# Mariachiar/Spatiotemporal-Deepfake-Detection-for-Live-Video-Calls

Measured on AMD Instinct MI355X. Metric: clips/sec (32x3x224x224), higher is better.
Workload: dtype bf16

## Files before the change

### spatiotemporal-deepfake-detection-for-live-video-calls_amd/csrc/af_conv111.hip

```cpp
#include "af_common.h"

namespace af {

struct C111Args {
    const char* in;
    const char* in2;
    const char* w;
    const char* w2;
    const float* scale;
    const float* shift;
    const char* res;
    char* out;
    int Cin, Cin2, Cout, out_ld, relu;
    int ncol;
    int T, HW, chunks;
    long long M;
    int tiles;
};

template <int NL, int NS, int D, int A = 0, int B = 0>
__device__ __forceinline__ void wait_counted(int nl, int ns) {
    if constexpr (A <= D - 1 && B <= D) {
        if (nl == A && ns == B) { wait_vmcnt<A * NL + B * NS>(); return; }
        if constexpr (B < D) wait_counted<NL, NS, D, A, B + 1>(nl, ns);
        else wait_counted<NL, NS, D, A + 1, 0>(nl, ns);
    } else {
        wait_vmcnt<0>();
    }
}

template <int DT, int KS1, int KS2, bool TPOOL, bool RES, int WC, int BM = 128, int NSLOT = 2>
__global__ __launch_bounds__(512, 1) void conv111_kernel(const C111Args a) {
    typedef Elem<DT> E;
    constexpr int EPC = E::EPC, ES = 16 / EPC;
    static_assert(EPC == 8, "16-bit storage types only");
    static_assert(WC == 64 || (WC == 32 && !TPOOL), "wave columns of 64 or 32 channels; the pooled tile order assumes 64");
    static_assert((BM == 128 || (BM == 64 && !TPOOL)) && NSLOT >= 2 && NSLOT <= 4, "tiles of 128 or 64 positions; the pooled row order assumes 128");
    constexpr int KS = KS1 + KS2, TN = WC / 16, D = NSLOT - 1;
    constexpr int NWN = 256 / WC, NWM = 8 / NWN, WPOS = BM / NWM, MT = WPOS / 16;
    constexpr int SLAB = BM * 128, STAGE = KS * SLAB;
    constexpr int PROW = WC + 4;
    constexpr int LPR = WC / 8, RPI = 64 / LPR, ITS = 16 / RPI;
    constexpr int NR = MT * ITS;
    constexpr int NPC = BM / 64;

    extern __shared__ uint4 smem[];
    const unsigned lds0 = (unsigned)(uintptr_t)(__attribute__((address_space(3))) char*)smem;
    const int tid = threadIdx.x, lane = tid & 63;
    const int wave = __builtin_amdgcn_readfirstlane(tid >> 6);
    const int frow = lane & 15, fg = lane >> 4;
    const int wn = wave % NWN, wm = wave / NWN;
    float* patch = reinterpret_cast<float*>(reinterpret_cast<char*>(smem) + NSLOT * STAGE) + wave * (16 * PROW);
    int col = blockIdx.x % a.ncol, first = blockIdx.x / a.ncol;
    const int stride = gridDim.x / a.ncol;
    if (gridDim.x % (8 * a.ncol) == 0) {
        const int xcd = blockIdx.x & 7, y = blockIdx.x >> 3;
        col = y % a.ncol;
        first = xcd + 8 * (y / a.ncol);
    }

    auto row_pixel = [&](int r) { return (r >> 6) * 32 + ((r >> 4) & 1) * 16 + (r & 15); };
    auto row_off = [&](int r) -> long long { return TPOOL ? (long long)((r >> 5) & 1) * a.HW + row_pixel(r) : r; };

    uint4 wreg[TN][2 * KS];
#pragma unroll
    for (int i = 0; i < TN; ++i) {
        const long long ch = col * 256 + wn * WC + i * 16 + frow;
#pragma unroll
        for (int k = 0; k < 2 * KS1; ++k)
            wreg[i][k] = *reinterpret_cast<const uint4*>(a.w + (ch * a.Cin + k * 32 + fg * 8) * ES);
#pragma unroll
        for (int k = 0; k < 2 * KS2; ++k)
            wreg[i][2 * KS1 + k] = *reinterpret_cast<const uint4*>(a.w2 + (ch * a.Cin2 + k * 32 + fg * 8) * ES);
    }

    constexpr bool REGEPI = WC == 32;
    const int rr = REGEPI ? frow : lane / LPR, cc = REGEPI ? (fg & 1) * 16 + (fg >> 1) * 8 : (lane % LPR) * 8;
    const int ch0 = col * 256 + wn * WC + cc;
    f32x4 sc[2], sf[2];
#pragma unroll
    for (int e = 0; e < 2; ++e) {
        const int chp = REGEPI ? col * 256 + wn * WC + e * 16 + fg * 4 : ch0 + 4 * e;
        sc[e] = *reinterpret_cast<const f32x4*>(a.scale + chp);
        sf[e] = *reinterpret_cast<const f32x4*>(a.shift + chp);
    }

    const int drow = lane >> 3, chunk = (lane & 7) ^ drow;
    const int xrow = wave * 8 + drow;
    const unsigned xoff = (unsigned)(row_off(xrow) * a.Cin * ES + chunk * 16);
    const unsigned x2off = KS2 ? (unsigned)(row_off(xrow) * a.Cin2 * ES + chunk * 16) : 0u;
    const int half_off = (int)(row_off(64) * a.Cin * ES), half2_off = (int)(row_off(64) * a.Cin2 * ES);
    auto tile_origin = [&](int tile, int& live) -> long long {
        if (TPOOL) {
            const int c = tile % a.chunks, nt = tile / a.chunks;
            live = a.HW - c * 64;
            return (long long)nt * 2 * a.HW + c * 64;
        }
        const long long o = (long long)tile * BM;
        live = (int)(a.M - o < BM ? a.M - o : BM);
        return o;
    };
    auto row_live = [&](int r, int live) { return TPOOL ? row_pixel(r) < live : r < live; };

    auto issue_tile = [&](int tile, int slot) {
        int live;
        const long long o = tile_origin(tile, live);
        const i32x4 d1 = make_desc(a.in + o * a.Cin * ES);
        const unsigned base = lds0 + slot * STAGE + wave * (8 * 128);
#pragma unroll
        for (int s = 0; s < KS1; ++s)
#pragma unroll
            for (int i = 0; i < NPC; ++i)
                blds16(row_live(xrow + 64 * i, live) ? xoff : kOutOfRange, d1, s * 128 + i * half_off, base + s * SLAB + i * (64 * 128));
        if (KS2) {
            const i32x4 d2 = make_desc(a.in2 + o * a.Cin2 * ES);
#pragma unroll
            for (int s = 0; s < KS2; ++s)
#pragma unroll
                for (int i = 0; i < NPC; ++i)
                    blds16(row_live(xrow + 64 * i, live) ? x2off : kOutOfRange, d2, s * 128 + i * half2_off, base + (KS1 + s) * SLAB + i * (64 * 128));
        }
    };
    const int row0 = wm * WPOS + rr;
    const unsigned res_lane = (unsigned)((row_off(row0) * a.Cout + ch0) * ES);
    const unsigned out_lane = (unsigned)(((long long)(TPOOL ? row_pixel(row0) : row0) * a.out_ld + ch0) * ES);
    auto k_row = [&](int k) { return (k / ITS) * 16 + (k % ITS) * RPI; };
    auto res_soff = [&](int k) { return (int)((row_off(k_row(k)) * a.Cout) * ES); };
    auto out_soff = [&](int k) { return (int)(((long long)(TPOOL ? row_pixel(k_row(k)) : k_row(k)) * a.out_ld) * ES); };
    auto load_residual = [&](int tile, u32x4 (&r)[NR]) {
        int live;
        const long long o = tile_origin(tile, live);
        const i32x4 rd = make_desc(a.res + o * a.Cout * ES);
#pragma unroll
        for (int k = 0; k < NR; ++k)
            r[k] = bload16_nt_uncounted(row_live(row0 + k_row(k), live) ? res_lane : kOutOfRange, rd, res_soff(k));
    };

    const int my_tiles = first < a.tiles ? (a.tiles - first + stride - 1) / stride : 0;
    u32x4 rs[NSLOT][NR];
#pragma unroll
    for (int u = 0; u < NSLOT; ++u)
#pragma unroll
        for (int k = 0; k < NR; ++k) rs[u][k] = u32x4{0u, 0u, 0u, 0u};
#pragma unroll
    for (int j = 0; j < D; ++j)
        if (j < my_tiles) {
            issue_tile(first + j * stride, j);
            if (RES) load_residual(first + j * stride, rs[j]);
        }
    __builtin_amdgcn_sched_barrier(0);
    constexpr int NL = KS * NPC + (RES ? NR : 0), NS = TPOOL ? NR / 2 : NR;
    static_assert((D - 1) * NL + D * NS <= 63, "vmcnt range");

    for (int q0 = 0; q0 < my_tiles; q0 += NSLOT) {
#pragma unroll
    for (int u = 0; u < NSLOT; ++u) {
        const int q = q0 + u;
        if (q >= my_tiles) break;
        const int tile = first + q * stride, slot = u;
        u32x4 (&rcur)[NR] = rs[u];
        if (D == 1) wait_vmcnt<0>();
        else {
            const int nl = my_tiles - 1 - q < D - 1 ? my_tiles - 1 - q : D - 1, ns = q < D ? q : D;
            wait_counted<NL, NS, D>(nl, ns);
        }
        __builtin_amdgcn_s_barrier();
        if (RES) {
#pragma unroll
            for (int k = 0; k < NR; ++k) asm volatile("" : "+v"(rcur[k]));
        }
        if (q + D < my_tiles) {
            issue_tile(tile + D * stride, (u + D) % NSLOT);
            if (RES) load_residual(tile + D * stride, rs[(u + D) % NSLOT]);
        }
        __builtin_amdgcn_sched_barrier(0);

        int live;
        const long long o = tile_origin(tile, live);
        const long long opos = TPOOL ? (o - o % a.HW) / 2 + o % a.HW : o;
        char* obase = a.out + opos * a.out_ld * ES;
        const uint4* xs = smem + slot * (STAGE / 16) + (wm * WPOS + frow) * 8;

#pragma unroll
        for (int h = 0; h < MT / 2; ++h) {
            f32x4 acc[TN][2];
#pragma unroll
            for (int i = 0; i < TN; ++i) { acc[i][0] = f32x4{0.f, 0.f, 0.f, 0.f}; acc[i][1] = f32x4{0.f, 0.f, 0.f, 0.f}; }
#pragma unroll
            for (int k = 0; k < 2 * KS; ++k) {
                const int c = ((k & 1) * 4 + fg) ^ (frow & 7);
                uint4 bf[2];
#pragma unroll
                for (int jl = 0; jl < 2; ++jl) bf[jl] = xs[(k >> 1) * (SLAB / 16) + (TPOOL ? h + 2 * jl : 2 * h + jl) * 16 * 8 + c];
#pragma unroll
                for (int i = 0; i < TN; ++i)
#pragma unroll
                    for (int jl = 0; jl < 2; ++jl) Mma<DT>::run(wreg[i][k], bf[jl], acc[i][jl]);
            }

            if constexpr (REGEPI) {
                const float lo = a.relu ? 0.f : -__builtin_inff();
#pragma unroll
                for (int jl = 0; jl < 2; ++jl) {
                    const int j = 2 * h + jl, row = wm * WPOS + j * 16 + rr;
                    f32x4 v0 = acc[0][jl] * sc[0] + sf[0], v1 = acc[1][jl] * sc[1] + sf[1];
                    if (RES) {
                        const u32x4 x = rcur[j];
                        const u32x2 s0 = __builtin_amdgcn_permlane16_swap(x[0], x[2], false, false);
                        const u32x2 s1 = __builtin_amdgcn_permlane16_swap(x[1], x[3], false, false);
                        const u32x2 ra = u32x2{s0[0], s1[0]}, rb = u32x2{s0[1], s1[1]};
                        v0 += Vec4<DT>::load(&ra); v1 += Vec4<DT>::load(&rb);
                    }
                    v0[0] = max_nan(v0[0], lo); v0[1] = max_nan(v0[1], lo); v0[2] = max_nan(v0[2], lo); v0[3] = max_nan(v0[3], lo);
                    v1[0] = max_nan(v1[0], lo); v1[1] = max_nan(v1[1], lo); v1[2] = max_nan(v1[2], lo); v1[3] = max_nan(v1[3], lo);
                    u32x2 p0, p1;
                    Vec4<DT>::store(&p0, v0); Vec4<DT>::store(&p1, v1);
                    const u32x4 o = swap_pair16(p0, p1);
                    if (row_live(row, live))
                        __builtin_nontemporal_store(o, reinterpret_cast<u32x4*>(obase + out_soff(j) + out_lane));
                }
                continue;
            }
            float keep[ITS][8];
#pragma unroll
            for (int jl = 0; jl < 2; ++jl) {
                const int j = TPOOL ? h + 2 * jl : 2 * h + jl;
#pragma unroll
                for (int i = 0; i < TN; ++i)
                    *reinterpret_cast<f32x4*>(patch + frow * PROW + i * 16 + fg * 4) = acc[i][jl];
                __builtin_amdgcn_wave_barrier();
#pragma unroll
                for (int it = 0; it < ITS; ++it) {
                    const int prow = it * RPI + rr, row = wm * WPOS + j * 16 + prow;
                    float v[8];
#pragma unroll
                    for (int e = 0; e < 8; e += 4) {
                        const f32x4 t = *reinterpret_cast<const f32x4*>(patch + prow * PROW + cc + e);
                        const f32x4 r = t * sc[e >> 2] + sf[e >> 2];
                        v[e] = r[0]; v[e + 1] = r[1]; v[e + 2] = r[2]; v[e + 3] = r[3];
                    }
                    if (RES) {
                        const uint4 rraw = __builtin_bit_cast(uint4, rcur[j * ITS + it]);
                        const typename E::type* re = reinterpret_cast<const typename E::type*>(&rraw);
#pragma unroll
                        for (int e = 0; e < 8; ++e) v[e] += E::to_f32(re[e]);
                    }
                    if (a.relu) {
#pragma unroll
                        for (int e = 0; e < 8; ++e) v[e] = relu_f(v[e]);
                    }
                    if (TPOOL && jl == 0) {
#pragma unroll
                        for (int e = 0; e < 8; ++e) keep[it][e] = v[e];
                        continue;
                    }
                    if (TPOOL) {
#pragma unroll
                        for (int e = 0; e < 8; ++e) v[e] = max_nan(keep[it][e], v[e]);
                    }
                    uint4 ov;
                    typename E::type* oe = reinterpret_cast<typename E::type*>(&ov);
#pragma unroll
                    for (int e = 0; e < 8; ++e) oe[e] = E::from_f32(v[e]);
                    if (row_live(row, live))
                        __builtin_nontemporal_store(__builtin_bit_cast(u32x4, ov), reinterpret_cast<u32x4*>(obase + out_soff(j * ITS + it) + out_lane));
                }
                __builtin_amdgcn_wave_barrier();
            }
        }
    }
    }
}

template <int DT, int KS1, int KS2, bool TPOOL, bool RES, int WC = 64, int BM = 128, int NSLOT = 2>
static int launch111(const C111Args& a, int blocks, hipStream_t stream) {
    const int lds = NSLOT * (KS1 + KS2) * BM * 128 + 8 * 16 * (WC + 4) * 4;
    AF_SET_MAX_LDS((&conv111_kernel<DT, KS1, KS2, TPOOL, RES, WC, BM, NSLOT>), lds, "conv111");
    hipLaunchKernelGGL((conv111_kernel<DT, KS1, KS2, TPOOL, RES, WC, BM, NSLOT>), dim3(blocks), dim3(512), lds, stream, a);
    AF_CHECK_LAUNCH("conv111_kernel");
    return AF_OK;
}

static int conv111_bm(const af_conv_desc* d) { return d->cin >= 128 ? 64 : 128; }

static long long conv111_tiles(const af_conv_desc* d, const af_conv_desc* d2, int out_ld) {
    if (d->dtype == AF_F32) return 0;
    if (d->kt != 1 || d->kh != 1 || d->kw != 1 || d->st != 1 || d->sh != 1 || d->sw != 1 || d->pt || d->ph || d->pw) return 0;
    if (d->cout % 256 != 0 || (d->tpool != 0 && d->tpool != 1)) return 0;
    if (d2) {
        if (d->cin != 64 || d2->cin != 64 || d->tpool) return 0;
        if (d2->st != 1 || d2->sh != 1 || d2->sw != 1 || d2->t != d->t || d2->h != d->h || d2->w != d->w) return 0;
    } else if (d->cin != 64 && d->cin != 128 && d->cin != 256) return 0;
    if (d->tpool && (d->cin != 64 || d->t % 2 != 0)) return 0;
    const long long hw = (long long)d->h * d->w;
    if ((hw + 128) * 128 * 2 * 2 >= (1LL << 31)) return 0;
    const int bm = conv111_bm(d);
    const long long tiles = d->tpool ? (long long)d->n * (d->t / 2) * ((hw + 63) / 64) : ((long long)d->n * d->t * hw + bm - 1) / bm;
    if (tiles >= (1LL << 30)) return 0;
    if (tiles * bm / 128 * (d->cout / 256) < 4LL * device_cus()) return 0;
    return tiles;
}

bool conv111_applies(const af_conv_desc* d, const af_conv_desc* d2, const void* residual, int out_ld) {
    if (d2 && residual) return false;
    return conv111_tiles(d, d2, out_ld) != 0;
}

int conv111_run(const af_conv_desc* d, const void* in, const void* w_packed, const af_conv_desc* d2, const void* in2,
                const void* w2_packed, const float* scale, const float* shift, const void* residual, void* out, int out_ld,
                hipStream_t stream) {
    C111Args a;
    a.in = (const char*)in; a.in2 = (const char*)in2; a.w = (const char*)w_packed; a.w2 = (const char*)w2_packed;
    a.scale = scale; a.shift = shift; a.res = (const char*)residual; a.out = (char*)out;
    a.Cin = d->cin; a.Cin2 = d2 ? d2->cin : 0; a.Cout = d->cout; a.out_ld = out_ld; a.relu = d->relu;
    a.ncol = d->cout / 256;
    a.T = d->t; a.HW = d->h * d->w; a.chunks = (a.HW + 63) / 64;
    a.M = (long long)d->n * d->t * a.HW;
    a.tiles = (int)conv111_tiles(d, d2, out_ld);
    int streams = device_cus() / a.ncol;
    if (streams > a.tiles) streams = a.tiles;
    const int blocks = streams * a.ncol;
    const bool bf = d->dtype == AF_BF16;
#define AF_C111(K1, K2, TP, RS) (bf ? launch111<AF_BF16, K1, K2, TP, RS>(a, blocks, stream) : launch111<AF_F16, K1, K2, TP, RS>(a, blocks, stream))
    if (d2) return AF_C111(1, 1, false, false);
    if (d->tpool) return residual ? AF_C111(1, 0, true, true) : AF_C111(1, 0, true, false);
    if (d->cin == 64) return residual ? AF_C111(1, 0, false, true) : AF_C111(1, 0, false, false);
    if (d->cin == 256) {
        if (env_int("AF_C111_WC64", 1) != 0)
            return residual ? (bf ? launch111<AF_BF16, 4, 0, false, true, 64, 64, 2>(a, blocks, stream) : launch111<AF_F16, 4, 0, false, true, 64, 64, 2>(a, blocks, stream))
                            : (bf ? launch111<AF_BF16, 4, 0, false, false, 64, 64, 2>(a, blocks, stream) : launch111<AF_F16, 4, 0, false, false, 64, 64, 2>(a, blocks, stream));
        return residual ? (bf ? launch111<AF_BF16, 4, 0, false, true, 32, 64, 4>(a, blocks, stream) : launch111<AF_F16, 4, 0, false, true, 32, 64, 4>(a, blocks, stream))
                        : (bf ? launch111<AF_BF16, 4, 0, false, false, 32, 64, 4>(a, blocks, stream) : launch111<AF_F16, 4, 0, false, false, 32, 64, 4>(a, blocks, stream));
    }
    return residual ? (bf ? launch111<AF_BF16, 2, 0, false, true, 64, 64, 4>(a, blocks, stream) : launch111<AF_F16, 2, 0, false, true, 64, 64, 4>(a, blocks, stream))
                    : (bf ? launch111<AF_BF16, 2, 0, false, false, 64, 64, 4>(a, blocks, stream) : launch111<AF_F16, 2, 0, false, false, 64, 64, 4>(a, blocks, stream));
#undef AF_C111
}

}
```

Measured before the change: 3499.

## Add narrow 1x1x1 conv kernel for 512-to-128 channel layers with register-resident weights

Adds a specialized persistent kernel for pointwise convolutions with 512 input and 128 output channels, a shape the existing kernel rejected because it requires cout divisible by 256. The full weight slice is held in registers per wave, activation tiles of 32 rows are streamed through a 4-slot LDS pipeline via buffer-to-LDS loads, and outputs are staged through an LDS patch for coalesced nontemporal stores. The intent is to move these layers off the slower fallback path. The cost is heavy register pressure from pinned weight fragments and a new code path to maintain.

```diff
diff --git a/spatiotemporal-deepfake-detection-for-live-video-calls_amd/csrc/af_conv111.hip b/spatiotemporal-deepfake-detection-for-live-video-calls_amd/csrc/af_conv111.hip
--- a/spatiotemporal-deepfake-detection-for-live-video-calls_amd/csrc/af_conv111.hip
+++ b/spatiotemporal-deepfake-detection-for-live-video-calls_amd/csrc/af_conv111.hip
@@ -279,6 +279,141 @@
     hipLaunchKernelGGL((conv111_kernel<DT, KS1, KS2, TPOOL, RES, WC, BM, NSLOT>), dim3(blocks), dim3(512), lds, stream, a);
     AF_CHECK_LAUNCH("conv111_kernel");
     return AF_OK;
+}
+
+template <int DT, int WC, int BM, int NSLOT>
+__global__ __launch_bounds__(512, 1) void conv111_narrow_kernel(const C111Args a) {
+    typedef Elem<DT> E;
+    static_assert(E::EPC == 8, "16-bit storage types only");
+    constexpr int K = 512, CO = 128, ROWB = K * 2, OROWB = CO * 2;
+    constexpr int TN = WC / 16, NWN = CO / WC, NWM = 8 / NWN, WPOS = BM / NWM, MT = WPOS / 16, D = NSLOT - 1;
+    static_assert((WC == 16 || WC == 32) && WPOS % 16 == 0 && MT >= 1 && BM % 8 == 0, "wave grid");
+    constexpr int STAGE = BM * ROWB, NL = BM / 8;
+    constexpr int PSTR = OROWB + 16;
+    constexpr int SB = BM * OROWB / 512, LPR = OROWB / SB, RPW = 64 / LPR;
+    static_assert((SB == 16 || SB == 8) && RPW * 8 == BM, "one store per wave and tile");
+    constexpr int NWAIT = (D - 1) * NL + D;
+    static_assert(NWAIT <= 63, "vmcnt range");
+
+    extern __shared__ uint4 smem[];
+    const unsigned lds0 = (unsigned)(uintptr_t)(__attribute__((address_space(3))) char*)smem;
+    char* const patch = reinterpret_cast<char*>(smem) + NSLOT * STAGE;
+    const int tid = threadIdx.x, lane = tid & 63;
+    const int wave = __builtin_amdgcn_readfirstlane(tid >> 6);
+    const int frow = lane & 15, fg = lane >> 4;
+    const int wn = wave % NWN, wm = wave / NWN;
+    const int first = blockIdx.x, stride = gridDim.x;
+    const int my_tiles = first < a.tiles ? (a.tiles - first + stride - 1) / stride : 0;
+
+    u32x4 wreg[TN][16];
+    f32x4 sc[TN], sf[TN];
+#pragma unroll
+    for (int i = 0; i < TN; ++i) {
+        const int ch = wn * WC + i * 16;
+#pragma unroll
+        for (int k = 0; k < 16; ++k)
+            wreg[i][k] = *reinterpret_cast<const u32x4*>(a.w + ((long long)(ch + frow) * K + k * 32 + fg * 8) * 2);
+        sc[i] = *reinterpret_cast<const f32x4*>(a.scale + ch + fg * 4);
+        sf[i] = *reinterpret_cast<const f32x4*>(a.shift + ch + fg * 4);
+    }
+#pragma unroll
+    for (int i = 0; i < TN; ++i) {
+#pragma unroll
+        for (int k = 0; k < 16; ++k) pin_frag(wreg[i][k]);
+        acc_live(sc[i]); acc_live(sf[i]);
+    }
+
+    unsigned xoff[2];
+#pragma unroll
+    for (int p = 0; p < 2; ++p) xoff[p] = (unsigned)((lane ^ ((wave + 8 * p) & 15)) * 16);
+    auto issue_tile = [&](int tile, int slot) {
+        const long long o = (long long)tile * BM;
+        const int live = tile < a.tiles ? (int)(a.M - o < BM ? a.M - o : BM) : 0;
+        const i32x4 d1 = make_desc(a.in + (live ? o : 0) * ROWB);
+        const unsigned base = lds0 + slot * STAGE + wave * ROWB;
+#pragma unroll
+        for (int i = 0; i < NL; ++i)
+            blds16_m0(wave + 8 * i < live ? xoff[i & 1] : kOutOfRange, d1, (wave + 8 * i) * ROWB, base + i * 8 * ROWB);
+    };
+    const unsigned xs_lane = (unsigned)((wm * WPOS + frow) * ROWB);
+    const unsigned pw_lane = (unsigned)((wm * WPOS + frow) * PSTR + (wn * WC + fg * 4) * 2);
+    const int srow = wave * RPW + lane / LPR, scol = (lane % LPR) * SB;
+    const unsigned pr_lane = (unsigned)(srow * PSTR + scol);
+    const unsigned out_lane = (unsigned)(((long long)srow * a.out_ld) * 2 + scol);
+    const float lo = a.relu ? 0.f : -__builtin_inff();
+
+#pragma unroll
+    for (int j = 0; j < D; ++j) issue_tile(first + j * stride, j);
+    __builtin_amdgcn_sched_barrier(0);
+
+    int slot = 0;
+    for (int q = 0; q < my_tiles; ++q) {
+        const int tile = first + q * stride;
+        if (q >= D) wait_vmcnt<NWAIT>();
+        else wait_vmcnt_dyn<NWAIT>((D - 1) * NL + q);
+        __builtin_amdgcn_s_barrier();
+        const int fill = slot == 0 ? NSLOT - 1 : slot - 1;
+        issue_tile(tile + D * stride, fill);
+        __builtin_amdgcn_sched_barrier(0);
+
+        const long long o = (long long)tile * BM;
+        const int live = (int)(a.M - o < BM ? a.M - o : BM);
+        const char* xs = reinterpret_cast<const char*>(smem) + slot * STAGE + xs_lane;
+        f32x4 acc[TN][MT];
+#pragma unroll
+        for (int i = 0; i < TN; ++i)
+#pragma unroll
+            for (int j = 0; j < MT; ++j) acc[i][j] = f32x4{0.f, 0.f, 0.f, 0.f};
+#pragma unroll
+        for (int k = 0; k < 16; ++k) {
+            const int c = (k * 4 + fg) ^ frow;
+#pragma unroll
+            for (int j = 0; j < MT; ++j) {
+                const uint4 bf = *reinterpret_cast<const uint4*>(xs + j * 16 * ROWB + c * 16);
+#pragma unroll
+                for (int i = 0; i < TN; ++i) Mma<DT>::run(__builtin_bit_cast(uint4, wreg[i][k]), bf, acc[i][j]);
+            }
+        }
+#pragma unroll
+        for (int i = 0; i < TN; ++i)
+#pragma unroll
+            for (int j = 0; j < MT; ++j) {
+                f32x4 v = acc[i][j] * sc[i] + sf[i];
+                v[0] = max_nan(v[0], lo); v[1] = max_nan(v[1], lo); v[2] = max_nan(v[2], lo); v[3] = max_nan(v[3], lo);
+                Vec4<DT>::store(patch + pw_lane + j * 16 * PSTR + i * 32, v);
+            }
+        wait_lgkmcnt<0>();
+        __builtin_amdgcn_s_barrier();
+        char* op = a.out + o * a.out_ld * 2 + out_lane;
+        if constexpr (SB == 16) {
+            const u32x4 ov = *reinterpret_cast<const u32x4*>(patch + pr_lane);
+            if (srow < live) __builtin_nontemporal_store(ov, reinterpret_cast<u32x4*>(op));
+        } else {
+            const u32x2 ov = *reinterpret_cast<const u32x2*>(patch + pr_lane);
+            if (srow < live) __builtin_nontemporal_store(ov, reinterpret_cast<u32x2*>(op));
+        }
+        slot = slot == NSLOT - 1 ? 0 : slot + 1;
+    }
+}
+
+template <int DT, int WC, int BM, int NSLOT>
+static int launch111n(const C111Args& a, int blocks, hipStream_t stream) {
+    const int lds = NSLOT * BM * 1024 + BM * (256 + 16);
+    AF_SET_MAX_LDS((&conv111_narrow_kernel<DT, WC, BM, NSLOT>), lds, "conv111 narrow");
+    hipLaunchKernelGGL((conv111_narrow_kernel<DT, WC, BM, NSLOT>), dim3(blocks), dim3(512), lds, stream, a);
+    AF_CHECK_LAUNCH("conv111_narrow_kernel");
+    return AF_OK;
+}
+
+constexpr int kNarrowBM = 32;
+static long long conv111_narrow_tiles(const af_conv_desc* d, const af_conv_desc* d2, const void* residual) {
+    if (d2 || residual || d->dtype == AF_F32 || d->tpool) return 0;
+    if (d->kt != 1 || d->kh != 1 || d->kw != 1 || d->st != 1 || d->sh != 1 || d->sw != 1 || d->pt || d->ph || d->pw) return 0;
+    if (d->cin != 512 || d->cout != 128) return 0;
+    const long long M = (long long)d->n * d->t * d->h * d->w, tiles = (M + kNarrowBM - 1) / kNarrowBM;
+    if (tiles >= (1LL << 30)) return 0;
+    if (M / 128 < 4LL * device_cus()) return 0;
+    return tiles;
 }
 
 static int conv111_bm(const af_conv_desc* d) { return d->cin >= 128 ? 64 : 128; }
@@ -303,6 +438,7 @@
 
 bool conv111_applies(const af_conv_desc* d, const af_conv_desc* d2, const void* residual, int out_ld) {
     if (d2 && residual) return false;
+    if (conv111_narrow_tiles(d, d2, residual)) return true;
     return conv111_tiles(d, d2, out_ld) != 0;
 }
 
@@ -316,6 +452,13 @@
     a.ncol = d->cout / 256;
     a.T = d->t; a.HW = d->h * d->w; a.chunks = (a.HW + 63) / 64;
     a.M = (long long)d->n * d->t * a.HW;
+    if (const long long nt = conv111_narrow_tiles(d, d2, residual)) {
+        a.tiles = (int)nt;
+        const long long per = (nt + device_cus() - 1) / device_cus();
+        const int blocks = (int)((nt + per - 1) / per);
+        return d->dtype == AF_BF16 ? launch111n<AF_BF16, 32, kNarrowBM, 4>(a, blocks, stream)
+                                   : launch111n<AF_F16, 32, kNarrowBM, 4>(a, blocks, stream);
+    }
     a.tiles = (int)conv111_tiles(d, d2, out_ld);
     int streams = device_cus() / a.ncol;
     if (streams > a.tiles) streams = a.tiles;
```

New measurement: 3503, median of 2. No clear change (+0.1%).
